# 3decomp/poissbox

Hardware: AMD Instinct MI355X
Metric: CG iter/s and DoF-updates/s at 512^3; achieved HBM GB/s vs peak (higher is better)
Workload: dtype f64

## Files before the change

poissbox_amd/csrc/pb_mg.cpp:

```cpp
#include <algorithm>
#include <cmath>

#include "pb_mg.hpp"

namespace pb {

int mg_plan_levels(const int64_t n[3], int nranks, int levels_req) {
  std::vector<int64_t> k0(nranks), nz(nranks);
  for (int r = 0; r < nranks; ++r) pb_slab_partition(n[2], nranks, r, &k0[r], &nz[r]);
  int64_t cur[3] = {n[0], n[1], n[2]};
  int L = 1;
  const int cap = levels_req > 0 ? levels_req : 64;
  while (L < cap) {
    bool ok = true;
    for (int d = 0; d < 3; ++d) ok = ok && cur[d] % 4 == 0;
    if (levels_req <= 0) ok = ok && std::min(cur[0], std::min(cur[1], cur[2])) > 4;
    for (int r = 0; r < nranks; ++r) ok = ok && k0[r] % 2 == 0 && nz[r] % 2 == 0;
    if (!ok) break;
    for (int d = 0; d < 3; ++d) cur[d] /= 2;
    for (int r = 0; r < nranks; ++r) {
      k0[r] /= 2;
      nz[r] /= 2;
    }
    ++L;
// ... 10 lines not shown
    if (L.own) pb_grid_destroy(L.g);
  if (mg->mem) (void)hipFree(mg->mem);
  if (mg->agg) (void)hipFree(mg->agg);
  if (mg->pmem) (void)hipFree(mg->pmem);
  if (mg->vmem) (void)hipFree(mg->vmem);
  delete mg;
}

static MgTune mg_tunings(const pb_ctx* ctx) {
  MgTune t;
  t.engine_min_plane = tune("mg_engine_min_plane", ctx->split ? 128 * 128 : 256 * 256);
  t.restrict_z_min_cols = tune("mg_restrict_z_min_cols", 4096);
  t.tail_max = tune("mg_tail_max", 8192);
  t.split_fused = tune("mg_split_fused", 1) != 0;
  t.poly_fused = tune("mg_poly_fused", 1) != 0;
  t.vc_pre_fused = tune("mg_varcoef_pre_fused", 1) != 0;
  t.vc_dinv_stored = tune("mg_varcoef_dinv_stored", 0) != 0;
  t.vc_kc = tune("mg_varcoef_kc", 0);
  return t;
}

static LevelPlan level_plan(const Mg* mg, int l, bool have_xs) {
  const MgTune& tn = mg->tn;
  const pb_grid* g = mg->lv[l].g;
  const bool split = mg->ctx->split;
  LevelPlan p;
  p.engine = g->plane >= tn.engine_min_plane;
  if (l + 1 >= (int)mg->lv.size()) return p;
  const pb_grid* c = mg->lv[l + 1].g;
  p.march = c->n[0] * c->n[1] >= tn.restrict_z_min_cols;
  if (mg->custom()) return p;
  const bool sweep2 = p.engine && sor_sweep2_supported(g);
  const bool u4 = sweep2 && (!split || (tn.split_fused && g->k0 % 2 == 0));
  if (u4 && g->nzl % 2 == 0 && (!split || g->nzl >= 3)) p.pre = LevelPlan::FusedRestrict;
  else if (sweep2) p.pre = LevelPlan::FusedResidual;
  if (u4 && have_xs && p.march && (!split || (g->nzl >= 2 && c->nzl >= 2)))
    p.post = LevelPlan::PostSweep;
  else if (sweep2 && p.march)
    p.post = LevelPlan::ProlongThenSweep2;
  return p;
}

static int tail_first(const Mg* mg) {
  const int L = (int)mg->lv.size();
  int Lt = L;
  for (int l = L - 1; l >= 1 && mg->lv[l].size() <= mg->tn.tail_max; --l) Lt = l;
  return L - Lt > kTailMax ? L : Lt;
}

static int mg_agglomerate_setup(Mg* mg) {
  pb_ctx* ctx = mg->ctx;
// ... 63 lines not shown
      lv.g = g;
      continue;
    }
    const int rc = grid_create_part(ctx, lv.n, g->L, g->k0 >> l, g->nzl >> l, &lv.g);
    if (rc != PB_OK) {
      mg_destroy(mg);
      return rc;
    }
    lv.own = true;
  }
  std::vector<double**> arrays;
  std::vector<int64_t> sizes;
  int64_t total = 0;
  for (int l = 0; l < L; ++l) {
    MgLevel& lv = mg->lv[l];
    const bool xs = level_plan(mg, l, true).post == LevelPlan::PostSweep;
    for (double** a : {l > 0 ? &lv.x : nullptr, l > 0 ? &lv.b : nullptr,
                       l < L - 1 ? &lv.res : nullptr, xs ? &lv.xs : nullptr}) {
      if (!a) continue;
      arrays.push_back(a);
      sizes.push_back(lv.g->nlocal);
      total += lv.g->nlocal;
    }
  }
  if (total > 0 && hipMalloc(&mg->mem, (size_t)total * sizeof(double)) != hipSuccess) {
    mg_destroy(mg);
    return set_error(PB_ERR_ALLOC, "multigrid levels: out of device memory");
  }
  double* p = mg->mem;
  for (size_t i = 0; i < arrays.size(); ++i) {
    *arrays[i] = p;
// ... 100 lines not shown
    PB_TRY(poly_step(mg, F, y, ypa, r, scale, omega, yo, ro));
    yp = y;
    y = yo;
    r = ro;
  }
  *ycur = const_cast<double*>(y);
  *rcur = const_cast<double*>(r);
  return PB_OK;
}

static int down_leg(Mg* mg, int l) {
  pb_ctx* ctx = mg->ctx;
  MgLevel& F = mg->lv[l];
  MgLevel& C = mg->lv[l + 1];
  const LevelPlan& p = F.plan;
  F.cur = p.post == LevelPlan::PostSweep ? F.xs : F.x;
  double* res = F.res;
  {
    ScopedTimer t1(ctx, l == 0 ? "mg_fine_smooth_first" : "mg_coarse_levels");
    if (p.pre == LevelPlan::FusedRestrict)
      return launch_presmooth_restrict(F.g, F.s, C.g, F.b, F.cur, C.b, mg->omega, mg->skip);
    if (p.pre == LevelPlan::FusedResidual) {
      PB_TRY(launch_presmooth_residual(F.g, F.s, F.b, F.cur, F.res, mg->omega, mg->skip));
    } else if (mg->poly()) {
      PB_TRY(poly_smooth(mg, F, true, &F.cur, &res));
    } else {
      PB_TRY(level_smooth(mg, F, 0, 1));
      for (int i = 1; i < mg->sm.nu; ++i) {
        PB_TRY(level_smooth(mg, F, 0, 0));
        PB_TRY(level_smooth(mg, F, 1, 0));
      }
// ... 85 lines not shown
```

poissbox_amd/csrc/pb_mg.hpp:

```cpp
#pragma once
#include <vector>

#include "pb_internal.hpp"

namespace pb {

struct MgGeo {
  int nx, ny, nzl;
  int64_t plane, nlocal, k0;
};

struct LevelPlan {
  enum Pre { FusedRestrict, FusedResidual, Sweeps };
  enum Post { PostSweep, ProlongThenSweep2, ProlongThenHalves };
  bool engine = false;
  Pre pre = Sweeps;
  Post post = ProlongThenHalves;
  bool march = false;
};

struct MgLevel {
  int64_t n[3];
  double h[3];
  Star s;
  pb_grid* g = nullptr;
  bool own = false;
  double* x = nullptr;
  double* b = nullptr;
  double* res = nullptr;
  double* xs = nullptr;
  double* t1 = nullptr;
  double* t2 = nullptr;
  double* r2 = nullptr;
// ... 3 lines not shown
  Star vs;
  LevelPlan plan;
  double* cur = nullptr;
  int64_t size() const { return n[0] * n[1] * n[2]; }
  MgGeo geo() const {
    return MgGeo{(int)g->n[0], (int)g->n[1], (int)g->nzl, g->plane, g->nlocal, g->k0};
  }
};

struct MgTune {
  int64_t engine_min_plane;
  int64_t restrict_z_min_cols;
  int64_t tail_max;
  bool split_fused;
  bool poly_fused;
  bool vc_pre_fused, vc_dinv_stored;
  int vc_kc;
};

struct MgSums {
  const CgState* st = nullptr;
  int* nparts = nullptr;
};

struct CoarsePlanes {
  const double *xc, *lo, *hi;
};

static constexpr int kTailMax = 12;

// ... 42 lines not shown
```

poissbox_amd/csrc/pb_mg_sweep.hip:

```cpp
#include <algorithm>
#include <type_traits>

#include "pb_device.hpp"

namespace pb {

#ifndef PB_SWEEP2_TY
#define PB_SWEEP2_TY 3
#endif
static constexpr int kTY2 = PB_SWEEP2_TY;
static constexpr int kRW = kTY2 + 4;
static constexpr int kSegOut = 112;
static constexpr int kSegLead = 4;

__device__ __forceinline__ double pick(bool e1, const double (&v)[2]) {
  const long long m = -(long long)e1;
  return __builtin_bit_cast(double, (__builtin_bit_cast(long long, v[1]) & m) |
                                        (__builtin_bit_cast(long long, v[0]) & ~m));
}

struct Sweep2Geo {
  int nx, ny, nzl;
  int64_t plane;
  int nseg, ntile, kc, nchunk;
// ... 362 lines not shown
      rq[0][r] = rq[1][r];
      rq[1][r] = rq[2][r];
      rq[2][r] = rn[r];
#pragma unroll
      for (int e = 0; e < 2; ++e) {
        s1[0][r][e] = s1[1][r][e];
        s1[1][r][e] = s1[2][r][e];
        bq[0][r][e] = bq[1][r][e];
        bq[1][r][e] = bq[2][r][e];
      }
    }
    keepb(nraw, bq[2]);
  }
}

template <int NW, int TY>
__device__ __forceinline__ void presmooth_restrict_u4_range(
    const Sweep2Geo& g, int ncx, int64_t cplane, double cx, double cy, double cz, double cc,
    double omega, const double* __restrict__ b, double* __restrict__ xout,
    double* __restrict__ bc, int seg, int tile, int kb, int ke, double (&xch)[2][8][NW][64]) {
  static_assert(TY % 2 == 0 && TY >= 2, "whole coarse rows per wave");
  constexpr int RB = NW * TY;
  constexpr int LO = 4;
  constexpr int SB = RB - 2 * LO;
  constexpr int NCR = TY / 2;
  const double icc = 1.0 / cc;
  const int lane = threadIdx.x & 63, wid = __builtin_amdgcn_readfirstlane(threadIdx.x >> 6);
  const int nx = g.nx, ny = g.ny, nz = g.nzl;
  if (kb >= nz) return;
  const int g0 = tile * SB - LO;
  const int br0 = wid * TY;
// ... 141 lines not shown
          a = a + cx * xl;
          a = a + cc * s1c[r][e];
          a = a + cx * xr;
          a = a + cy * yp;
          a = a + cz * s1p[r][e];
          rv[e] = bq0[r][e] - a;
        }
        const double rlo = dpp_from_lower(rv[1]);
        const double rhi = dpp_from_upper(rv[0]);
        double sx = w[0] * rlo;
        sx = sx + w[1] * rv[0];
        sx = sx + w[2] * rv[1];
        sx = sx + w[3] * rhi;
        sxc[r] = sx;
      }
      if (k >= kb && k < ke && out_ok) {
        const int64_t base = (int64_t)k * g.plane;
#pragma unroll
        for (int r = 0; r < TY; ++r)
          if (row_ok >> r & 1u) store_row<2>(xout, rix(base + ro[r]), s1c[r], g.nt);
      }
    } else {
#pragma unroll
      for (int r = 0; r < TY; ++r) sxc[r] = 0.0;
    }
    xch[KP][6][wid][lane] = sxc[0];
    xch[KP][7][wid][lane] = sxc[TY - 1];
    const int kr = k - 1;
    if (kr >= kb - 1) {
#pragma unroll
      for (int c = 0; c < NCR; ++c) {
        double sy = 0.0;
#pragma unroll
        for (int bb = 0; bb < 4; ++bb) {
          const int r = 2 * c - 1 + bb;
// ... 15 lines not shown
      }
    }
    redv(std::integral_constant<int, KP ^ 1>{}, raw, rn);
    xch[KP][0][wid][lane] = rn[0];
    xch[KP][1][wid][lane] = rn[TY - 1];
  };
#pragma unroll 1
  for (int k = kb - 3; k <= ke + 1; k += 4) {
    body(std::integral_constant<int, 0>{}, k);
    body(std::integral_constant<int, 1>{}, k + 1);
    body(std::integral_constant<int, 2>{}, k + 2);
    body(std::integral_constant<int, 3>{}, k + 3);
  }
}

template <class F>
__device__ __forceinline__ void split_ranges(const Sweep2Geo& g, int bid, F&& fn) {
  const int ncol = g.nseg * g.ntile, W = g.wsplit, T = g.nzl / W;
  if (bid < T * ncol) {
    const int kb = (bid / ncol) * W;
    fn(bid % ncol, kb, kb + W);
    return;
  }
  const int k0 = T * W, h = g.nzl - k0;
  if (h <= 0) return;
  const int64_t total = (int64_t)ncol * h;
  const int64_t e = min(total, (int64_t)(bid - T * ncol + 1) * W);
  for (int64_t s = (int64_t)(bid - T * ncol) * W; s < e;) {
    const int col = (int)(s / h);
    const int kb = (int)(s - (int64_t)col * h);
    const int ke = (int)min((int64_t)h, kb + (e - s));
    fn(col, k0 + kb, k0 + ke);
    s += ke - kb;
  }
}

template <int NW, int TY>
__global__ __launch_bounds__(64 * NW) void presmooth_restrict_u4_kernel(
    Sweep2Geo g, int ncx, int64_t cplane, double cx, double cy, double cz, double cc,
    double omega, const double* __restrict__ b, double* __restrict__ xout,
    double* __restrict__ bc, const int* skip) {
  __shared__ double xch[2][8][NW][64];
  if (skip && *skip) return;
  int bid = xcd_block(g.remap);
  if (g.wsplit > 0) {
    split_ranges(g, bid, [&](int col, int kb, int ke) {
      presmooth_restrict_u4_range<NW, TY>(g, ncx, cplane, cx, cy, cz, cc, omega, b, xout, bc,
                                          col % g.nseg, col / g.nseg, kb, ke, xch);
      __syncthreads();
    });
    return;
  }
  const int seg = bid % g.nseg;
  bid /= g.nseg;
  const int tile = bid % g.ntile;
  const int chunk = bid / g.ntile;
  const int kb = chunk * g.kc;
  presmooth_restrict_u4_range<NW, TY>(g, ncx, cplane, cx, cy, cz, cc, omega, b, xout, bc, seg,
                                      tile, kb, min(kb + g.kc, g.nzl), xch);
}

struct PostGeo {
  int ncx, ncy, ncz;
  int64_t cplane;
  int split;
  const double* cgh[4];
};

template <bool SUMS, int NW, int TY>
__device__ __forceinline__ void post_sweep_u4_range(
    const Sweep2Geo& g, const PostGeo& cgeo, double cx, double cy, double cz, double cc,
    double omega, const double* __restrict__ xs, const double* __restrict__ xc,
    const double* __restrict__ b, double* __restrict__ xout, double mu, int seg, int tile, int kb,
    int ke, double (&xch)[2][6][NW][64], double (&acc)[4]) {
  static_assert(TY % 2 == 0 && TY >= 2, "own rows start on an even fine row");
  constexpr int RB = NW * TY;
  constexpr int SB = RB - 4;
  constexpr int NC = TY / 2 + 2;
  const double icc = 1.0 / cc;
  const int lane = threadIdx.x & 63, wid = __builtin_amdgcn_readfirstlane(threadIdx.x >> 6);
  const int nx = g.nx, ny = g.ny, nz = g.nzl;
  if (kb < nz) {
    const int g0 = tile * SB - 2;
    const int br0 = wid * TY;
    const int j0 = g0 + br0;
    auto wrap = [](int v, int n) { v %= n; return v < 0 ? v + n : v; };
    int ip = seg * kSegOut + 2 * (lane - kSegLead);
    if (ip < 0) ip += nx;
    if (ip >= nx) ip -= nx;
    const int o = seg * kSegOut + 2 * (lane - kSegLead);
    const bool out_ok = lane >= kSegLead && lane < kSegLead + kSegOut / 2 && o < nx;
    int64_t ro[TY];
    unsigned row_ok = 0;
#pragma unroll
    for (int r = 0; r < TY; ++r) {
      ro[r] = (int64_t)wrap(j0 + r, ny) * nx;
      const int brow = br0 + r;
      if (brow >= 2 && brow < RB - 2 && g0 + brow < ny) row_ok |= 1u << r;
    }
    const unsigned boff = (unsigned)ip * 8u;
    auto rix = [&](int64_t row) { return RowIx{row, boff}; };
    auto wrapk = [&](int kk) { kk %= nz; return kk < 0 ? kk + nz : kk; };
    auto pl = [&](int kk) -> int64_t { return (int64_t)wrapk(kk) * g.plane; };
    int64_t crow[NC];
#pragma unroll
    for (int t = 0; t < NC; ++t) crow[t] = (int64_t)wrap((j0 >> 1) - 1 + t, cgeo.ncy) * cgeo.ncx;
    const unsigned cboff = (unsigned)(ip >> 1) * 8u;
    auto xsplane = [&](int kk) -> const double* {
      if (!g.split) return xs + pl(kk);
      if (kk >= 0 && kk < nz) return xs + (int64_t)kk * g.plane;
      const int gi = kk < 0 ? max(kk + 2, 0) : 2 + min(kk - nz, 1);
      return g.xg + (int64_t)gi * g.plane;
    };
    auto ldx = [&](double (&dst)[TY + 2][2], int kk) {
      const double* src = xsplane(kk);
#pragma unroll
      for (int r = 0; r < TY; ++r) load_row<2>(src, rix(ro[r]), dst[r + 1]);
    };
    auto ldc = [&](double (&cv)[NC], int K) {
      const double* cp;
      if (!cgeo.split) {
        K %= cgeo.ncz;
        if (K < 0) K += cgeo.ncz;
        cp = xc + (int64_t)K * cgeo.cplane;
      } else if (K >= 0 && K < cgeo.ncz) {
        cp = xc + (int64_t)K * cgeo.cplane;
      } else {
        const int gi = K < 0 ? max(K + 2, 0) : 2 + min(K - cgeo.ncz, 1);
        cp = cgeo.cgh[gi];
      }
#pragma unroll
      for (int t = 0; t < NC; ++t)
        cv[t] = *reinterpret_cast<const double*>(reinterpret_cast<const char*>(cp + crow[t]) + cboff);
    };
    auto yinterp = [&](const double (&cv)[NC], double (&Y)[TY][2]) {
      double xi[NC][2];
#pragma unroll
      for (int t = 0; t < NC; ++t) {
        const double c = cv[t];
        xi[t][0] = 0.75 * c + 0.25 * dpp_from_lower(c);
        xi[t][1] = 0.75 * c + 0.25 * dpp_from_upper(c);
      }
#pragma unroll
      for (int r = 0; r < TY; ++r) {
        const int tJ = 1 + (r >> 1);
        const int tf = (r & 1) ? tJ + 1 : tJ - 1;
#pragma unroll
        for (int e = 0; e < 2; ++e) Y[r][e] = 0.75 * xi[tJ][e] + 0.25 * xi[tf][e];
      }
    };
    auto prolong = [&](double (&v)[TY + 2][2], const double (&Yn)[TY][2],
                       const double (&Yf)[TY][2]) {
#pragma unroll
      for (int r = 0; r < TY; ++r)
#pragma unroll
        for (int e = 0; e < 2; ++e) v[r + 1][e] = v[r + 1][e] + (0.75 * Yn[r][e] + 0.25 * Yf[r][e]);
    };
    auto ldb = [&](double (&dst)[TY][2], int kk) {
      const double* src = !g.split ? b + pl(kk)
                          : (kk >= 0 && kk < nz ? b + (int64_t)kk * g.plane
                                                : (kk < 0 ? g.bg_lo : g.bg_hi));
#pragma unroll
      for (int r = 0; r < TY; ++r) load_row<2>(src, rix(ro[r]), dst[r]);
    };
    auto e1 = [](int r, int P) { return ((r + P) & 1) ^ 1; };
    auto half1 = [&](auto Pc, const double (&zmv)[TY], const double (&xcn)[TY + 2][2],
                     const double (&xp)[TY + 2][2], const double (&bb)[TY][2],
                     double (&out)[TY]) {
      constexpr int P = decltype(Pc)::value;
#pragma unroll
      for (int r = 0; r < TY; ++r) {
        const int e = e1(r, P);
        const double xl = e ? xcn[r + 1][0] : dpp_from_lower(xcn[r + 1][1]);
        const double xr = e ? dpp_from_upper(xcn[r + 1][0]) : xcn[r + 1][1];
        double nb = cz * zmv[r];
        nb = nb + cy * xcn[r][e];
        nb = nb + cx * xl;
        nb = nb + cx * xr;
        nb = nb + cy * xcn[r + 2][e];
        nb = nb + cz * xp[r + 1][e];
        const double t = (bb[r][e] - nb) * icc;
        out[r] = (1.0 - omega) * xcn[r + 1][e] + omega * t;
      }
    };
    auto half2 = [&](auto Pc, int kk, const double (&sm)[TY], const double (&sc)[TY],
                     const double (&sp)[TY], const double (&sh)[2], const double (&xo)[TY],
                     const double (&bo)[TY], const double (&bc1)[SUMS ? TY : 1]) {
      constexpr int P = decltype(Pc)::value;
      const int64_t base = pl(kk);
#pragma unroll
      for (int r = 0; r < TY; ++r) {
        const int e2 = e1(r, P) ^ 1;
        const double cself = sc[r];
        const double xl = e2 ? cself : dpp_from_lower(cself);
        const double xr = e2 ? dpp_from_upper(cself) : cself;
        double nb = cz * sm[r];
        nb = nb + cy * (r == 0 ? sh[0] : sc[r == 0 ? 0 : r - 1]);
        nb = nb + cx * xl;
        nb = nb + cx * xr;
        nb = nb + cy * (r == TY - 1 ? sh[1] : sc[r == TY - 1 ? r : r + 1]);
        nb = nb + cz * sp[r];
        const double t = (bo[r] - nb) * icc;
        const double v = (1.0 - omega) * xo[r] + omega * t;
        double ov[2];
        ov[e2] = v;
        ov[e2 ^ 1] = cself;
        if (out_ok && (row_ok >> r & 1u)) {
          store_row<2>(xout, rix(base + ro[r]), ov, g.nt);
          if constexpr (SUMS) {
            double rv2[2];
            rv2[e2] = bo[r];
            rv2[e2 ^ 1] = bc1[r];
#pragma unroll
            for (int e = 0; e < 2; ++e) {
              const double t2 = ov[e] - mu;
              acc[0] += t2;
              acc[1] += t2 * t2;
              acc[2] += t2 * rv2[e];
              acc[3] += rv2[e];
            }
          }
        }
      }
    };
    const int wm = wid > 0 ? wid - 1 : wid, wp = wid < NW - 1 ? wid + 1 : wid;
    auto put_x = [&](int par, const double (&v)[TY + 2][2]) {
      xch[par][0][wid][lane] = v[1][0];
      xch[par][1][wid][lane] = v[1][1];
      xch[par][2][wid][lane] = v[TY][0];
      xch[par][3][wid][lane] = v[TY][1];
    };
    double XQ[2][TY + 2][2];
    double XM[2][TY];
    double S1[4][TY];
    double SH[2][2];
    double BB[2][TY];
    double BB1[2][SUMS ? TY : 1];
    double YC[2][TY][2];
    const int K0 = kb >> 1;
    {
      double cv[NC];
      ldc(cv, K0 - 2);
      yinterp(cv, YC[0]);
      ldc(cv, K0 - 1);
      yinterp(cv, YC[1]);
      ldx(XQ[1], kb - 2);
      prolong(XQ[1], YC[1], YC[0]);
#pragma unroll
      for (int r = 0; r < TY; ++r) XM[1][r] = XQ[1][r + 1][e1(r, 0) ^ 1];
      ldc(cv, K0);
      yinterp(cv, YC[0]);
      ldx(XQ[0], kb - 1);
      prolong(XQ[0], YC[1], YC[0]);
      put_x(1, XQ[0]);
    }
#pragma unroll
    for (int r = 0; r < TY; ++r) {
      XM[0][r] = BB[0][r] = BB[1][r] = 0.0;
      S1[0][r] = S1[1][r] = S1[2][r] = 0.0;
      if constexpr (SUMS) BB1[0][r] = BB1[1][r] = 0.0;
    }
    SH[0][0] = SH[0][1] = 0.0;
    auto body = [&](auto Qc, int k) {
      constexpr int Q = decltype(Qc)::value;
      constexpr int KP = Q & 1;
      double (&xq1)[TY + 2][2] = XQ[Q & 1];
      double (&xq2)[TY + 2][2] = XQ[(Q + 1) & 1];
      double (&xm)[TY] = XM[Q & 1];
      double (&x0)[TY] = XM[(Q + 1) & 1];
      double (&bm)[TY] = BB[Q & 1];
      double (&bm1)[SUMS ? TY : 1] = BB1[Q & 1];
      double (&shp)[2] = SH[Q & 1];
      double (&shc)[2] = SH[(Q + 1) & 1];
      constexpr int KN = Q >> 1;
      double bq1[TY][2], cv[NC];
      ldx(xq2, k + 2);
      if constexpr (Q & 1) ldc(cv, ((k + 2) >> 1) + 1);
      ldb(bq1, k + 1);
      __syncthreads();
      {
        constexpr int rp = KP ^ 1;
        xq1[0][0] = xch[rp][2][wm][lane];
        xq1[0][1] = xch[rp][3][wm][lane];
        xq1[TY + 1][0] = xch[rp][0][wp][lane];
        xq1[TY + 1][1] = xch[rp][1][wp][lane];
        shc[0] = xch[rp][5][wm][lane];
        shc[1] = xch[rp][4][wp][lane];
      }
      if (k > kb && k <= ke)
        half2(std::integral_constant<int, KP ^ 1>{}, k - 1, S1[Q], S1[(Q + 1) & 3],
              S1[(Q + 2) & 3], shp, xm, bm, bm1);
      if constexpr (Q & 1) yinterp(cv, YC[KN ^ 1]);
      prolong(xq2, YC[KN], YC[KN ^ 1]);
      put_x(KP, xq2);
      double (&s1n)[TY] = S1[(Q + 3) & 3];
      half1(std::integral_constant<int, KP ^ 1>{}, x0, xq1, xq2, bq1, s1n);
      xch[KP][4][wid][lane] = s1n[0];
      xch[KP][5][wid][lane] = s1n[TY - 1];
#pragma unroll
      for (int r = 0; r < TY; ++r) {
        const int e = e1(r, KP ^ 1);
        xm[r] = xq1[r + 1][e ^ 1];
        bm[r] = bq1[r][e ^ 1];
        if constexpr (SUMS) bm1[r] = bq1[r][e];
      }
    };
#pragma unroll 1
    for (int k = kb - 2; k <= ke; k += 4) {
      body(std::integral_constant<int, 0>{}, k);
      body(std::integral_constant<int, 1>{}, k + 1);
      body(std::integral_constant<int, 2>{}, k + 2);
      body(std::integral_constant<int, 3>{}, k + 3);
    }
  }
}

template <bool SUMS, int NW, int TY>
__global__ __launch_bounds__(64 * NW) void post_sweep_u4_kernel(
    Sweep2Geo g, PostGeo cgeo, double cx, double cy, double cz, double cc, double omega,
    const double* __restrict__ xs, const double* __restrict__ xc, const double* __restrict__ b,
    double* __restrict__ xout, const CgState* st, double* parts, const int* skip) {
  __shared__ double xch[2][6][NW][64];
  if (skip && *skip) return;
  double acc[4] = {0.0, 0.0, 0.0, 0.0};
  const double mu = SUMS ? st->mu : 0.0;
  int bid = xcd_block(g.remap);
  if (g.wsplit > 0) {
    split_ranges(g, bid, [&](int col, int kb, int ke) {
      post_sweep_u4_range<SUMS, NW, TY>(g, cgeo, cx, cy, cz, cc, omega, xs, xc, b, xout, mu,
                                        col % g.nseg, col / g.nseg, kb, ke, xch, acc);
      __syncthreads();
    });
  } else {
    const int seg = bid % g.nseg;
    bid /= g.nseg;
    const int tile = bid % g.ntile;
    const int chunk = bid / g.ntile;
    const int kb = chunk * g.kc;
    post_sweep_u4_range<SUMS, NW, TY>(g, cgeo, cx, cy, cz, cc, omega, xs, xc, b, xout, mu, seg,
                                      tile, kb, min(kb + g.kc, g.nzl), xch, acc);
  }
  if constexpr (SUMS) block_partials<4>(acc, parts);
}

bool sor_sweep2_supported(const pb_grid* g) {
  return g->n[0] >= 128 && g->n[0] % 2 == 0 && g->n[1] % 2 == 0 && g->n[1] >= 8 &&
         g->nzl >= 4 && tune("mg_sweep2", 1) != 0;
}

static int ensure_ghost2(pb_grid* g) {
  if (!g->ghost2 && hipMalloc(&g->ghost2, 6 * (size_t)g->plane * sizeof(double)) != hipSuccess)
    return set_error(PB_ERR_ALLOC, "deep ghost planes: out of device memory");
  return PB_OK;
}

// ... 91 lines not shown
  if (g->k0 % 2 != 0) return set_error(PB_ERR_UNSUPPORTED, "%s: odd slab origin", what);
  sweep2_geo(g, geo);
  geo.split = 0;
  geo.xg = geo.bg_lo = geo.bg_hi = nullptr;
  geo.ntile = (geo.ny + rows - 1) / rows;
  return PB_OK;
}

int launch_post_sweep(pb_grid* g, const Star& s, const pb_grid* cg, const double* xs,
                      const double* xc, const double* b, double* xout, double omega,
                      const int* skip, const CgState* sums_st, int* nparts,
                      const double* xc_full) {
  ScopedTimer tm(g->ctx, "mg_post_sweep");
  const bool split = g->ctx->split;
  if (xs == xout) return set_error(PB_ERR_ARG, "fused post-smoothing must run out of place");
  constexpr int nw = 8, ty = 4;
  Sweep2Geo geo;
  PB_TRY(u4_setup("fused post-smoothing", g, cg, 2, "fused post-smoothing: slabs of < 2 planes",
                  nw * ty - 4, geo));
  PostGeo cgeo{(int)cg->n[0], (int)cg->n[1], (int)cg->nzl, cg->plane, 0,
                {nullptr, nullptr, nullptr, nullptr}};
  if (split) {
    pb_grid* gc = const_cast<pb_grid*>(cg);
    PB_TRY(ensure_ghost2(g));
    PB_TRY(ensure_ghost2(gc));
    PB_TRY(halo_exchange_n(g, xs, xs + (g->nzl - 2) * g->plane, 2, g->ghost2,
                           g->ghost2 + 2 * g->plane));
    PB_TRY(halo_exchange(g, b, b + (g->nzl - 1) * g->plane));
    geo.split = 1;
    geo.xg = g->ghost2;
// ... 9 lines not shown
    } else {
      PB_TRY(halo_exchange_n(gc, xc, xc + (gc->nzl - 2) * gc->plane, 2, gc->ghost2,
                             gc->ghost2 + 2 * gc->plane));
      for (int i = 0; i < 4; ++i) cgeo.cgh[i] = gc->ghost2 + (int64_t)i * gc->plane;
    }
  }
  const int columns = geo.nseg * geo.ntile;
  const int target = 8 * g->ctx->num_cus;
  int nchunk = std::max(1, (target + columns - 1) / columns);
  const int minz = std::min(64, std::max(16, geo.nzl / 8));
  nchunk = std::min(nchunk, std::max(1, geo.nzl / minz));
  int64_t nblocks = set_chunks(geo, nchunk, 4);
  nblocks = balanced_split(g, geo, std::max(0, tune("mg_u4_split", 0)), 4, nblocks);
  double* parts;
  PB_TRY(sums_parts(g, sums_st, nblocks, nparts, &parts));
  auto kern = sums_st ? post_sweep_u4_kernel<true, nw, ty> : post_sweep_u4_kernel<false, nw, ty>;
  hipLaunchKernelGGL(kern, dim3((unsigned)nblocks), dim3(64 * nw), 0, g->ctx->stream, geo, cgeo,
                     s.cx, s.cy, s.cz, s.cc, omega, xs, xc, b, xout, sums_st, parts, skip);
  PB_HIP(hipGetLastError());
  return PB_OK;
}

int launch_presmooth_restrict(pb_grid* g, const Star& s, const pb_grid* cg, const double* b,
                              double* xout, double* bc, double omega, const int* skip) {
  ScopedTimer tm(g->ctx, "mg_presmooth_restrict");
  const bool split = g->ctx->split;
  if (b == xout) return set_error(PB_ERR_ARG, "fused pre-smoothing must run out of place");
  if (!sor_sweep2_supported(g) || g->nzl % 2)
    return set_error(PB_ERR_UNSUPPORTED, "fused restriction: grid not supported");
  constexpr int nw = 8, ty = 4;
  Sweep2Geo geo;
// ... 2 lines not shown
  if (split) {
    PB_TRY(ensure_ghost2(g));
    PB_TRY(halo_exchange_n(g, b, b + (g->nzl - 3) * g->plane, 3, g->ghost2,
                           g->ghost2 + 3 * g->plane));
    geo.split = 1;
    geo.xg = g->ghost2;
  }
  const int columns = geo.nseg * geo.ntile;
  int nchunk = std::max(1, g->ctx->num_cus / columns);
  if (geo.nzl / nchunk < 128) nchunk = std::max(1, (4 * g->ctx->num_cus + columns - 1) / columns);
  nchunk = std::min(nchunk, std::max(1, geo.nzl / 16));
  int64_t nblocks = set_chunks(geo, nchunk, 2);
  const int ps = tune("mg_u4_split", -1);
  nblocks = balanced_split(g, geo, ps >= 0 ? ps : (nblocks > g->ctx->num_cus ? 1 : 0), 2,
                           nblocks);
  hipLaunchKernelGGL((presmooth_restrict_u4_kernel<nw, ty>), dim3((unsigned)nblocks),
                     dim3(64 * nw), 0, g->ctx->stream, geo, (int)cg->n[0], cg->plane, s.cx, s.cy,
                     s.cz, s.cc, omega, b, xout, bc, skip);
  PB_HIP(hipGetLastError());
  return PB_OK;
}

int launch_presmooth_residual(pb_grid* g, const Star& s, const double* b, double* x, double* res,
                              double omega, const int* skip) {
  ScopedTimer tm(g->ctx, "mg_presmooth_residual");
  if (b == x || b == res || x == res)
    return set_error(PB_ERR_ARG, "fused pre-smoothing + residual must run out of place");
  Sweep2Geo geo;
  const int64_t nblocks = sweep2_geo(g, geo);
  PB_TRY(sweep2_ghosts(g, b, b, geo));
  auto kern = geo.split ? presmooth_resid_kernel<true> : presmooth_resid_kernel<false>;
  hipLaunchKernelGGL(kern, dim3((unsigned)nblocks), dim3(kThreads), 0, g->ctx->stream, geo,
                     s.cx, s.cy, s.cz, s.cc, omega, b, x, res, skip);
// ... 6 lines not shown
```

poissbox_amd/csrc/pb_runtime.cpp:

```cpp
#include <time.h>

#include <algorithm>
#include <atomic>
#include <chrono>
#include <cstdarg>
#include <cstdlib>
#include <cstring>
#include <condition_variable>
#include <memory>
#include <mutex>
#include <string>
#include <thread>
#include <unordered_map>

#include "pb_internal.hpp"

namespace pb {

hipError_t field_alloc(void** p, size_t bytes) { return hipMalloc(p, bytes); }

void field_free(void* p) {
  if (p) (void)hipFree(p);
}

namespace {
const char* const kTuneNames[] = {
    "a2a_copy_self", "cg_defer_x", "engine_kc_skew", "cg_fold", "cg_fuse", "cg_sr_fused", "cheb_fused", "comm_mark_every",
    "comm_stall_test_ms", "compact_lines", "fft_rupd", "fgmres_fused", "pipecg_fused", "fft_zpad", "fft_zpad_min_plane",
    "force_comm", "ksp_lazy0", "mg_agglomerate", "mg_engine_min_plane", "mg_poly_fused", "mg_restrict_z_min_cols",
    "mg_split_fused", "mg_sweep2", "mg_tail_max", "mg_u4_split", "mg_varcoef_dinv_stored", "mg_varcoef_kc",
    "mg_varcoef_pre_fused", "pcr_lines", "rich_fused", "sor_omega_any", "sr_ddiff",
    "stencil_kc", "stencil_kc_skew", "stencil_nt", "stencil_tall", "stencil_wgcu", "varcoef_dot_fused", "varcoef_wgcu", "x_dot_cu"};
constexpr int kNumTune = (int)(sizeof(kTuneNames) / sizeof(kTuneNames[0]));
std::atomic<int> g_tune_val[kNumTune];
std::atomic<int> g_tune_set[kNumTune];
std::atomic<int> g_tune_nset{0};
int tune_index(const char* name) {
  for (int i = 0; i < kNumTune; ++i)
    if (strcmp(kTuneNames[i], name) == 0) return i;
  return -1;
}
}

int tune(const char* name, int dflt) {
// ... 1019 lines not shown
```

Before: 102.4 billion.

## Recompute pre-smoothed iterate in post-sweep instead of storing it

On single-rank levels using the fused presmooth+restrict path, the pre-smoothed iterate x_s is no longer written to memory. The post-sweep kernel instead rebuilds it from b, since x starts at zero and one red-black sweep pass can be re-derived locally. This removes one full-grid store and one full-grid load per level per V-cycle and also frees the x_s buffer. In exchange the post-sweep does more arithmetic, more LDS exchange and an extra staging buffer, with scalar-load tricks to limit register pressure.

```diff
diff --git a/poissbox_amd/csrc/pb_mg.cpp b/poissbox_amd/csrc/pb_mg.cpp
--- a/poissbox_amd/csrc/pb_mg.cpp
+++ b/poissbox_amd/csrc/pb_mg.cpp
@@ -48,6 +48,7 @@
   t.tail_max = tune("mg_tail_max", 8192);
   t.split_fused = tune("mg_split_fused", 1) != 0;
   t.poly_fused = tune("mg_poly_fused", 1) != 0;
+  t.recompute_xs = tune("mg_recompute_xs", 1) != 0;
   t.vc_pre_fused = tune("mg_varcoef_pre_fused", 1) != 0;
   t.vc_dinv_stored = tune("mg_varcoef_dinv_stored", 0) != 0;
   t.vc_kc = tune("mg_varcoef_kc", 0);
@@ -68,7 +69,8 @@
   const bool u4 = sweep2 && (!split || (tn.split_fused && g->k0 % 2 == 0));
   if (u4 && g->nzl % 2 == 0 && (!split || g->nzl >= 3)) p.pre = LevelPlan::FusedRestrict;
   else if (sweep2) p.pre = LevelPlan::FusedResidual;
-  if (u4 && have_xs && p.march && (!split || (g->nzl >= 2 && c->nzl >= 2)))
+  p.recompute_xs = tn.recompute_xs && u4 && !split && p.pre == LevelPlan::FusedRestrict && p.march;
+  if (u4 && (have_xs || p.recompute_xs) && p.march && (!split || (g->nzl >= 2 && c->nzl >= 2)))
     p.post = LevelPlan::PostSweep;
   else if (sweep2 && p.march)
     p.post = LevelPlan::ProlongThenSweep2;
@@ -162,7 +164,8 @@
   int64_t total = 0;
   for (int l = 0; l < L; ++l) {
     MgLevel& lv = mg->lv[l];
-    const bool xs = level_plan(mg, l, true).post == LevelPlan::PostSweep;
+    const LevelPlan lp = level_plan(mg, l, true);
+    const bool xs = lp.post == LevelPlan::PostSweep && !lp.recompute_xs;
     for (double** a : {l > 0 ? &lv.x : nullptr, l > 0 ? &lv.b : nullptr,
                        l < L - 1 ? &lv.res : nullptr, xs ? &lv.xs : nullptr}) {
       if (!a) continue;
@@ -293,7 +296,7 @@
   MgLevel& F = mg->lv[l];
   MgLevel& C = mg->lv[l + 1];
   const LevelPlan& p = F.plan;
-  F.cur = p.post == LevelPlan::PostSweep ? F.xs : F.x;
+  F.cur = p.post == LevelPlan::PostSweep ? (p.recompute_xs ? nullptr : F.xs) : F.x;
   double* res = F.res;
   {
     ScopedTimer t1(ctx, l == 0 ? "mg_fine_smooth_first" : "mg_coarse_levels");
diff --git a/poissbox_amd/csrc/pb_mg.hpp b/poissbox_amd/csrc/pb_mg.hpp
--- a/poissbox_amd/csrc/pb_mg.hpp
+++ b/poissbox_amd/csrc/pb_mg.hpp
@@ -17,6 +17,7 @@
   Pre pre = Sweeps;
   Post post = ProlongThenHalves;
   bool march = false;
+  bool recompute_xs = false;
 };
 
 struct MgLevel {
@@ -50,6 +51,7 @@
   int64_t tail_max;
   bool split_fused;
   bool poly_fused;
+  bool recompute_xs;
   bool vc_pre_fused, vc_dinv_stored;
   int vc_kc;
 };
diff --git a/poissbox_amd/csrc/pb_mg_sweep.hip b/poissbox_amd/csrc/pb_mg_sweep.hip
--- a/poissbox_amd/csrc/pb_mg_sweep.hip
+++ b/poissbox_amd/csrc/pb_mg_sweep.hip
@@ -400,7 +400,7 @@
   }
 }
 
-template <int NW, int TY>
+template <bool STORE, int NW, int TY>
 __device__ __forceinline__ void presmooth_restrict_u4_range(
     const Sweep2Geo& g, int ncx, int64_t cplane, double cx, double cy, double cz, double cc,
     double omega, const double* __restrict__ b, double* __restrict__ xout,
@@ -572,11 +572,13 @@
         sx = sx + w[3] * rhi;
         sxc[r] = sx;
       }
-      if (k >= kb && k < ke && out_ok) {
-        const int64_t base = (int64_t)k * g.plane;
-#pragma unroll
-        for (int r = 0; r < TY; ++r)
-          if (row_ok >> r & 1u) store_row<2>(xout, rix(base + ro[r]), s1c[r], g.nt);
+      if constexpr (STORE) {
+        if (k >= kb && k < ke && out_ok) {
+          const int64_t base = (int64_t)k * g.plane;
+#pragma unroll
+          for (int r = 0; r < TY; ++r)
+            if (row_ok >> r & 1u) store_row<2>(xout, rix(base + ro[r]), s1c[r], g.nt);
+        }
       }
     } else {
 #pragma unroll
@@ -622,7 +624,7 @@
   }
 }
 
-template <class F>
+template <bool PER_RANGE = false, class F>
 __device__ __forceinline__ void split_ranges(const Sweep2Geo& g, int bid, F&& fn) {
   const int ncol = g.nseg * g.ntile, W = g.wsplit, T = g.nzl / W;
   if (bid < T * ncol) {
@@ -630,11 +632,13 @@
     fn(bid % ncol, kb, kb + W);
     return;
   }
-  const int k0 = T * W, h = g.nzl - k0;
+  const int k0 = T * W;
+  int h = g.nzl - k0;
   if (h <= 0) return;
   const int64_t total = (int64_t)ncol * h;
   const int64_t e = min(total, (int64_t)(bid - T * ncol + 1) * W);
   for (int64_t s = (int64_t)(bid - T * ncol) * W; s < e;) {
+    if constexpr (PER_RANGE) asm volatile("" : "+s"(h));
     const int col = (int)(s / h);
     const int kb = (int)(s - (int64_t)col * h);
     const int ke = (int)min((int64_t)h, kb + (e - s));
@@ -643,7 +647,7 @@
   }
 }
 
-template <int NW, int TY>
+template <bool STORE, int NW, int TY>
 __global__ __launch_bounds__(64 * NW) void presmooth_restrict_u4_kernel(
     Sweep2Geo g, int ncx, int64_t cplane, double cx, double cy, double cz, double cc,
     double omega, const double* __restrict__ b, double* __restrict__ xout,
@@ -653,7 +657,7 @@
   int bid = xcd_block(g.remap);
   if (g.wsplit > 0) {
     split_ranges(g, bid, [&](int col, int kb, int ke) {
-      presmooth_restrict_u4_range<NW, TY>(g, ncx, cplane, cx, cy, cz, cc, omega, b, xout, bc,
+      presmooth_restrict_u4_range<STORE, NW, TY>(g, ncx, cplane, cx, cy, cz, cc, omega, b, xout, bc,
                                           col % g.nseg, col / g.nseg, kb, ke, xch);
       __syncthreads();
     });
@@ -664,7 +668,7 @@
   const int tile = bid % g.ntile;
   const int chunk = bid / g.ntile;
   const int kb = chunk * g.kc;
-  presmooth_restrict_u4_range<NW, TY>(g, ncx, cplane, cx, cy, cz, cc, omega, b, xout, bc, seg,
+  presmooth_restrict_u4_range<STORE, NW, TY>(g, ncx, cplane, cx, cy, cz, cc, omega, b, xout, bc, seg,
                                       tile, kb, min(kb + g.kc, g.nzl), xch);
 }
 
@@ -675,17 +679,30 @@
   const double* cgh[4];
 };
 
-template <bool SUMS, int NW, int TY>
+static constexpr int post_xch_slots(bool rx) { return rx ? 8 : 6; }
+static constexpr int post_park_len(bool rx, int nw, int ty) { return rx ? 2 * ty * 2 * nw * 64 : 1; }
+
+template <bool SUMS, bool RX, int NW, int TY>
 __device__ __forceinline__ void post_sweep_u4_range(
     const Sweep2Geo& g, const PostGeo& cgeo, double cx, double cy, double cz, double cc,
     double omega, const double* __restrict__ xs, const double* __restrict__ xc,
     const double* __restrict__ b, double* __restrict__ xout, double mu, int seg, int tile, int kb,
-    int ke, double (&xch)[2][6][NW][64], double (&acc)[4]) {
+    int ke, double (&xch)[2][post_xch_slots(RX)][NW][64],
+    double (&park)[post_park_len(RX, NW, TY)], double (&acc)[4]) {
   static_assert(TY % 2 == 0 && TY >= 2, "own rows start on an even fine row");
+  static_assert(!RX || (NW >= 2 && kSegLead >= 3), "recomputed x_s: two end waves, three halo pairs");
   constexpr int RB = NW * TY;
   constexpr int SB = RB - 4;
   constexpr int NC = TY / 2 + 2;
   const double icc = 1.0 / cc;
+  auto sdouble = [](double v) {
+    if constexpr (!RX) return v;
+    const unsigned long long u = __builtin_bit_cast(unsigned long long, v);
+    const unsigned lo = __builtin_amdgcn_readfirstlane((unsigned)u);
+    const unsigned hi = __builtin_amdgcn_readfirstlane((unsigned)(u >> 32));
+    return __builtin_bit_cast(double, ((unsigned long long)hi << 32) | lo);
+  };
+  const double om1 = sdouble(1.0 - omega), om1z = sdouble((1.0 - omega) * 0.0);
   const int lane = threadIdx.x & 63, wid = __builtin_amdgcn_readfirstlane(threadIdx.x >> 6);
   const int nx = g.nx, ny = g.ny, nz = g.nzl;
   if (kb < nz) {
@@ -708,7 +725,38 @@
     }
     const unsigned boff = (unsigned)ip * 8u;
     auto rix = [&](int64_t row) { return RowIx{row, boff}; };
-    auto wrapk = [&](int kk) { kk %= nz; return kk < 0 ? kk + nz : kk; };
+    auto srow = [](const double* p) {
+      const unsigned long long a = reinterpret_cast<unsigned long long>(p);
+      const unsigned lo = __builtin_amdgcn_readfirstlane((unsigned)a);
+      const unsigned hi = __builtin_amdgcn_readfirstlane((unsigned)(a >> 32));
+      return ((unsigned long long)hi << 32) | lo;
+    };
+    auto ld1_s = [](unsigned long long row, unsigned off) {
+      return *(const __attribute__((address_space(1))) double*)(row + off);
+    };
+    auto ld2_s = [](unsigned long long row, unsigned off, double (&v)[2]) {
+      const dv2 t = *(const __attribute__((address_space(1))) dv2*)(row + off);
+      v[0] = t.x;
+      v[1] = t.y;
+    };
+    auto st2_s = [](unsigned long long row, unsigned off, const double (&v)[2], int nt) {
+      dv2 t;
+      t.x = v[0];
+      t.y = v[1];
+      auto* q = (__attribute__((address_space(1))) dv2*)(row + off);
+      if (nt) __builtin_nontemporal_store(t, q);
+      else *q = t;
+    };
+    auto wrap3 = [](int v, int n) {
+      v = v < 0 ? v + n : v;
+      v = v >= n ? v - n : v;
+      return v >= n ? v - n : v;
+    };
+    auto wrapk = [&](int kk) {
+      if constexpr (RX) return wrap3(kk, nz);
+      kk %= nz;
+      return kk < 0 ? kk + nz : kk;
+    };
     auto pl = [&](int kk) -> int64_t { return (int64_t)wrapk(kk) * g.plane; };
     int64_t crow[NC];
 #pragma unroll
@@ -727,7 +775,9 @@
     };
     auto ldc = [&](double (&cv)[NC], int K) {
       const double* cp;
-      if (!cgeo.split) {
+      if (RX) {
+        cp = xc + (int64_t)wrap3(K, cgeo.ncz) * cgeo.cplane;
+      } else if (!cgeo.split) {
         K %= cgeo.ncz;
         if (K < 0) K += cgeo.ncz;
         cp = xc + (int64_t)K * cgeo.cplane;
@@ -738,8 +788,11 @@
         cp = cgeo.cgh[gi];
       }
 #pragma unroll
-      for (int t = 0; t < NC; ++t)
-        cv[t] = *reinterpret_cast<const double*>(reinterpret_cast<const char*>(cp + crow[t]) + cboff);
+      for (int t = 0; t < NC; ++t) {
+        const double* rowp = cp + crow[t];
+        if constexpr (RX) cv[t] = ld1_s(srow(rowp), cboff);
+        else cv[t] = *reinterpret_cast<const double*>(reinterpret_cast<const char*>(rowp) + cboff);
+      }
     };
     auto yinterp = [&](const double (&cv)[NC], double (&Y)[TY][2]) {
       double xi[NC][2];
@@ -769,10 +822,54 @@
                           : (kk >= 0 && kk < nz ? b + (int64_t)kk * g.plane
                                                 : (kk < 0 ? g.bg_lo : g.bg_hi));
 #pragma unroll
-      for (int r = 0; r < TY; ++r) load_row<2>(src, rix(ro[r]), dst[r]);
+      for (int r = 0; r < TY; ++r) {
+        if constexpr (RX) ld2_s(srow(src + ro[r]), boff, dst[r]);
+        else load_row<2>(src, rix(ro[r]), dst[r]);
+      }
     };
     auto e1 = [](int r, int P) { return ((r + P) & 1) ^ 1; };
-    auto half1 = [&](auto Pc, const double (&zmv)[TY], const double (&xcn)[TY + 2][2],
+    auto redval = [&](double bv) {
+      const double t = (bv - 0.0) * icc;
+      return om1z + omega * t;
+    };
+    auto redv = [&](auto Pc, const double (&v)[TY][2], double (&red)[TY]) {
+      constexpr int P = decltype(Pc)::value;
+#pragma unroll
+      for (int r = 0; r < TY; ++r) red[r] = redval(v[r][e1(r, P) ^ 1]);
+    };
+    auto xs_form = [&](auto Pc, auto Red, const double (&rm)[TY], const double (&rc)[TY],
+                       const double (&rp)[TY], const double (&rh)[2], const double (&bb)[TY][2],
+                       double (&out)[TY + 2][2]) {
+      constexpr int P = decltype(Pc)::value;
+#pragma unroll
+      for (int r = 0; r < TY; ++r) {
+        const int be = e1(r, P);
+        const double xl = be ? rc[r] : dpp_from_lower(rc[r]);
+        const double xr = be ? dpp_from_upper(rc[r]) : rc[r];
+        double nb = cz * rm[r];
+        nb = nb + cy * (r == 0 ? rh[0] : rc[r == 0 ? 0 : r - 1]);
+        nb = nb + cx * xl;
+        nb = nb + cx * xr;
+        nb = nb + cy * (r == TY - 1 ? rh[1] : rc[r == TY - 1 ? r : r + 1]);
+        nb = nb + cz * rp[r];
+        const double t = (bb[r][be] - nb) * icc;
+        const double v = om1z + omega * t;
+        if constexpr (decltype(Red)::value) out[r + 1][1 - be] = rc[r];
+        out[r + 1][be] = v;
+      }
+    };
+    const int64_t exrow =
+        (int64_t)wrap(wid == 0 ? j0 - 1 : (wid == NW - 1 ? j0 + TY : j0), ny) * nx;
+    auto ldex = [&](auto Pc, int kk) {
+      constexpr int P = decltype(Pc)::value;
+      const int e = P ? (wid == NW - 1 ? 1 : 0) : (wid == 0 ? 1 : 0);
+      return ld1_s(srow(b + pl(kk) + exrow + e), boff);
+    };
+    auto red_halo = [&](double (&rh)[2], double lo, double hi, double ex) {
+      rh[0] = wid == 0 ? redval(ex) : lo;
+      rh[1] = wid == NW - 1 ? redval(ex) : hi;
+    };
+    auto half1 =[&](auto Pc, const double (&zmv)[TY], const double (&xcn)[TY + 2][2],
                      const double (&xp)[TY + 2][2], const double (&bb)[TY][2],
                      double (&out)[TY]) {
       constexpr int P = decltype(Pc)::value;
@@ -788,7 +885,7 @@
         nb = nb + cy * xcn[r + 2][e];
         nb = nb + cz * xp[r + 1][e];
         const double t = (bb[r][e] - nb) * icc;
-        out[r] = (1.0 - omega) * xcn[r + 1][e] + omega * t;
+        out[r] = om1 * xcn[r + 1][e] + omega * t;
       }
     };
     auto half2 = [&](auto Pc, int kk, const double (&sm)[TY], const double (&sc)[TY],
@@ -809,12 +906,13 @@
         nb = nb + cy * (r == TY - 1 ? sh[1] : sc[r == TY - 1 ? r : r + 1]);
         nb = nb + cz * sp[r];
         const double t = (bo[r] - nb) * icc;
-        const double v = (1.0 - omega) * xo[r] + omega * t;
+        const double v = om1 * xo[r] + omega * t;
         double ov[2];
         ov[e2] = v;
         ov[e2 ^ 1] = cself;
         if (out_ok && (row_ok >> r & 1u)) {
-          store_row<2>(xout, rix(base + ro[r]), ov, g.nt);
+          if constexpr (RX) st2_s(srow(xout + base + ro[r]), boff, ov, g.nt);
+          else store_row<2>(xout, rix(base + ro[r]), ov, g.nt);
           if constexpr (SUMS) {
             double rv2[2];
             rv2[e2] = bo[r];
@@ -845,6 +943,7 @@
     double BB[2][TY];
     double BB1[2][SUMS ? TY : 1];
     double YC[2][TY][2];
+    double BQ[RX ? 4 : 1][TY][2];
     const int K0 = kb >> 1;
     {
       double cv[NC];
@@ -852,13 +951,39 @@
       yinterp(cv, YC[0]);
       ldc(cv, K0 - 1);
       yinterp(cv, YC[1]);
-      ldx(XQ[1], kb - 2);
+      if constexpr (RX) {
+        std::integral_constant<int, 0> ev;
+        std::integral_constant<int, 1> od;
+        double r3[TY], r2[TY], r1[TY], r0[TY], rh2[2], rh1[2];
+        ldb(BQ[2], kb - 3);
+        ldb(BQ[3], kb - 2);
+        ldb(BQ[0], kb - 1);
+        ldb(BQ[1], kb);
+        const double ex2 = ldex(ev, kb - 2), ex1 = ldex(od, kb - 1);
+        redv(od, BQ[2], r3);
+        redv(ev, BQ[3], r2);
+        redv(od, BQ[0], r1);
+        redv(ev, BQ[1], r0);
+        xch[0][6][wid][lane] = r2[0];
+        xch[0][7][wid][lane] = r2[TY - 1];
+        xch[0][4][wid][lane] = r1[0];
+        xch[0][5][wid][lane] = r1[TY - 1];
+        xch[1][6][wid][lane] = r0[0];
+        xch[1][7][wid][lane] = r0[TY - 1];
+        __syncthreads();
+        red_halo(rh2, xch[0][7][wm][lane], xch[0][6][wp][lane], ex2);
+        red_halo(rh1, xch[0][5][wm][lane], xch[0][4][wp][lane], ex1);
+        xs_form(ev, std::true_type{}, r3, r2, r1, rh2, BQ[3], XQ[1]);
+        xs_form(od, std::true_type{}, r2, r1, r0, rh1, BQ[0], XQ[0]);
+      } else {
+        ldx(XQ[1], kb - 2);
+      }
       prolong(XQ[1], YC[1], YC[0]);
 #pragma unroll
       for (int r = 0; r < TY; ++r) XM[1][r] = XQ[1][r + 1][e1(r, 0) ^ 1];
       ldc(cv, K0);
       yinterp(cv, YC[0]);
-      ldx(XQ[0], kb - 1);
+      if constexpr (!RX) ldx(XQ[0], kb - 1);
       prolong(XQ[0], YC[1], YC[0]);
       put_x(1, XQ[0]);
     }
@@ -881,12 +1006,21 @@
       double (&shp)[2] = SH[Q & 1];
       double (&shc)[2] = SH[(Q + 1) & 1];
       constexpr int KN = Q >> 1;
-      double bq1[TY][2], cv[NC];
-      ldx(xq2, k + 2);
+      double bql[RX ? 1 : TY][2], cv[NC];
+      double (&bq1)[TY][2] = *[&]() {
+        if constexpr (RX) return &BQ[Q];
+        else return &bql;
+      }();
+      double ex = 0.0, rh[2] = {0.0, 0.0};
+      if constexpr (RX) {
+        ldb(BQ[(Q + 2) & 3], k + 3);
+      } else {
+        ldx(xq2, k + 2);
+      }
       if constexpr (Q & 1) ldc(cv, ((k + 2) >> 1) + 1);
-      ldb(bq1, k + 1);
+      if constexpr (!RX) ldb(bq1, k + 1);
       __syncthreads();
-      {
+      auto get_halos = [&]() {
         constexpr int rp = KP ^ 1;
         xq1[0][0] = xch[rp][2][wm][lane];
         xq1[0][1] = xch[rp][3][wm][lane];
@@ -894,23 +1028,76 @@
         xq1[TY + 1][1] = xch[rp][1][wp][lane];
         shc[0] = xch[rp][5][wm][lane];
         shc[1] = xch[rp][4][wp][lane];
-      }
-      if (k > kb && k <= ke)
+      };
+      if constexpr (!RX) get_halos();
+      if constexpr (RX) {
+        if (k > kb && k <= ke) {
+          double pb2[TY], pb1[SUMS ? TY : 1];
+#pragma unroll
+          for (int r = 0; r < TY; ++r) {
+            pb2[r] = park[(((Q & 1) * TY + r) * 2 + 0) * (NW * 64) + threadIdx.x];
+            if constexpr (SUMS) pb1[r] = park[(((Q & 1) * TY + r) * 2 + 1) * (NW * 64) + threadIdx.x];
+          }
+          half2(std::integral_constant<int, KP ^ 1>{}, k - 1, S1[Q], S1[(Q + 1) & 3],
+                S1[(Q + 2) & 3], shp, xm, pb2, pb1);
+        }
+      } else if (k > kb && k <= ke) {
         half2(std::integral_constant<int, KP ^ 1>{}, k - 1, S1[Q], S1[(Q + 1) & 3],
               S1[(Q + 2) & 3], shp, xm, bm, bm1);
-      if constexpr (Q & 1) yinterp(cv, YC[KN ^ 1]);
-      prolong(xq2, YC[KN], YC[KN ^ 1]);
-      put_x(KP, xq2);
+      }
       double (&s1n)[TY] = S1[(Q + 3) & 3];
-      half1(std::integral_constant<int, KP ^ 1>{}, x0, xq1, xq2, bq1, s1n);
-      xch[KP][4][wid][lane] = s1n[0];
-      xch[KP][5][wid][lane] = s1n[TY - 1];
-#pragma unroll
-      for (int r = 0; r < TY; ++r) {
-        const int e = e1(r, KP ^ 1);
-        xm[r] = xq1[r + 1][e ^ 1];
-        bm[r] = bq1[r][e ^ 1];
-        if constexpr (SUMS) bm1[r] = bq1[r][e];
+      if constexpr (RX) {
+        __builtin_amdgcn_sched_barrier(0);
+        if constexpr (Q & 1) yinterp(cv, YC[KN ^ 1]);
+        const double (&Yn)[TY][2] = YC[KN];
+        const double (&Yf)[TY][2] = YC[KN ^ 1];
+        double rm[TY], rc[TY], rn[TY];
+        redv(std::integral_constant<int, KP>{}, BQ[(Q + 1) & 3], rc);
+#pragma unroll
+        for (int r = 0; r < TY; ++r) {
+          const int re = e1(r, KP) ^ 1;
+          xq2[r + 1][re] = rc[r] + (0.75 * Yn[r][re] + 0.25 * Yf[r][re]);
+        }
+        get_halos();
+        ex = ldex(std::integral_constant<int, KP>{}, k + 2);
+        half1(std::integral_constant<int, KP ^ 1>{}, x0, xq1, xq2, bq1, s1n);
+        xch[KP][4][wid][lane] = s1n[0];
+        xch[KP][5][wid][lane] = s1n[TY - 1];
+        redv(std::integral_constant<int, KP ^ 1>{}, bq1, rm);
+#pragma unroll
+        for (int r = 0; r < TY; ++r) {
+          const int e = e1(r, KP ^ 1);
+          xm[r] = xq1[r + 1][e ^ 1];
+          park[(((Q & 1) * TY + r) * 2 + 0) * (NW * 64) + threadIdx.x] = bq1[r][e ^ 1];
+          if constexpr (SUMS) park[(((Q & 1) * TY + r) * 2 + 1) * (NW * 64) + threadIdx.x] = bq1[r][e];
+        }
+        __builtin_amdgcn_sched_barrier(0);
+        red_halo(rh, xch[KP ^ 1][7][wm][lane], xch[KP ^ 1][6][wp][lane], ex);
+        redv(std::integral_constant<int, KP ^ 1>{}, BQ[(Q + 2) & 3], rn);
+        xch[KP][6][wid][lane] = rn[0];
+        xch[KP][7][wid][lane] = rn[TY - 1];
+        xs_form(std::integral_constant<int, KP>{}, std::false_type{}, rm, rc, rn, rh,
+                BQ[(Q + 1) & 3], xq2);
+#pragma unroll
+        for (int r = 0; r < TY; ++r) {
+          const int be = e1(r, KP);
+          xq2[r + 1][be] = xq2[r + 1][be] + (0.75 * Yn[r][be] + 0.25 * Yf[r][be]);
+        }
+        put_x(KP, xq2);
+      } else {
+        if constexpr (Q & 1) yinterp(cv, YC[KN ^ 1]);
+        prolong(xq2, YC[KN], YC[KN ^ 1]);
+        put_x(KP, xq2);
+        half1(std::integral_constant<int, KP ^ 1>{}, x0, xq1, xq2, bq1, s1n);
+        xch[KP][4][wid][lane] = s1n[0];
+        xch[KP][5][wid][lane] = s1n[TY - 1];
+#pragma unroll
+        for (int r = 0; r < TY; ++r) {
+          const int e = e1(r, KP ^ 1);
+          xm[r] = xq1[r + 1][e ^ 1];
+          bm[r] = bq1[r][e ^ 1];
+          if constexpr (SUMS) bm1[r] = bq1[r][e];
+        }
       }
     };
 #pragma unroll 1
@@ -923,20 +1110,23 @@
   }
 }
 
-template <bool SUMS, int NW, int TY>
+template <bool SUMS, bool RX, int NW, int TY>
 __global__ __launch_bounds__(64 * NW) void post_sweep_u4_kernel(
     Sweep2Geo g, PostGeo cgeo, double cx, double cy, double cz, double cc, double omega,
     const double* __restrict__ xs, const double* __restrict__ xc, const double* __restrict__ b,
     double* __restrict__ xout, const CgState* st, double* parts, const int* skip) {
-  __shared__ double xch[2][6][NW][64];
+  __shared__ double xch[2][post_xch_slots(RX)][NW][64];
+  __shared__ double park[post_park_len(RX, NW, TY)];
   if (skip && *skip) return;
   double acc[4] = {0.0, 0.0, 0.0, 0.0};
   const double mu = SUMS ? st->mu : 0.0;
   int bid = xcd_block(g.remap);
   if (g.wsplit > 0) {
-    split_ranges(g, bid, [&](int col, int kb, int ke) {
-      post_sweep_u4_range<SUMS, NW, TY>(g, cgeo, cx, cy, cz, cc, omega, xs, xc, b, xout, mu,
-                                        col % g.nseg, col / g.nseg, kb, ke, xch, acc);
+    split_ranges<RX>(g, bid, [&](int col, int kb, int ke) {
+      int nseg = g.nseg;
+      if constexpr (RX) asm volatile("" : "+s"(nseg));
+      post_sweep_u4_range<SUMS, RX, NW, TY>(g, cgeo, cx, cy, cz, cc, omega, xs, xc, b, xout, mu,
+                                            col % nseg, col / nseg, kb, ke, xch, park, acc);
       __syncthreads();
     });
   } else {
@@ -945,8 +1135,8 @@
     const int tile = bid % g.ntile;
     const int chunk = bid / g.ntile;
     const int kb = chunk * g.kc;
-    post_sweep_u4_range<SUMS, NW, TY>(g, cgeo, cx, cy, cz, cc, omega, xs, xc, b, xout, mu, seg,
-                                      tile, kb, min(kb + g.kc, g.nzl), xch, acc);
+    post_sweep_u4_range<SUMS, RX, NW, TY>(g, cgeo, cx, cy, cz, cc, omega, xs, xc, b, xout, mu, seg,
+                                      tile, kb, min(kb + g.kc, g.nzl), xch, park, acc);
   }
   if constexpr (SUMS) block_partials<4>(acc, parts);
 }
@@ -1068,6 +1258,8 @@
   ScopedTimer tm(g->ctx, "mg_post_sweep");
   const bool split = g->ctx->split;
   if (xs == xout) return set_error(PB_ERR_ARG, "fused post-smoothing must run out of place");
+  if (!xs && split)
+    return set_error(PB_ERR_UNSUPPORTED, "fused post-smoothing without x_s: one rank only");
   constexpr int nw = 8, ty = 4;
   Sweep2Geo geo;
   PB_TRY(u4_setup("fused post-smoothing", g, cg, 2, "fused post-smoothing: slabs of < 2 planes",
@@ -1107,7 +1299,10 @@
   nblocks = balanced_split(g, geo, std::max(0, tune("mg_u4_split", 0)), 4, nblocks);
   double* parts;
   PB_TRY(sums_parts(g, sums_st, nblocks, nparts, &parts));
-  auto kern = sums_st ? post_sweep_u4_kernel<true, nw, ty> : post_sweep_u4_kernel<false, nw, ty>;
+  auto kern = xs ? (sums_st ? post_sweep_u4_kernel<true, false, nw, ty>
+                            : post_sweep_u4_kernel<false, false, nw, ty>)
+                 : (sums_st ? post_sweep_u4_kernel<true, true, nw, ty>
+                            : post_sweep_u4_kernel<false, true, nw, ty>);
   hipLaunchKernelGGL(kern, dim3((unsigned)nblocks), dim3(64 * nw), 0, g->ctx->stream, geo, cgeo,
                      s.cx, s.cy, s.cz, s.cc, omega, xs, xc, b, xout, sums_st, parts, skip);
   PB_HIP(hipGetLastError());
@@ -1140,9 +1335,10 @@
   const int ps = tune("mg_u4_split", -1);
   nblocks = balanced_split(g, geo, ps >= 0 ? ps : (nblocks > g->ctx->num_cus ? 1 : 0), 2,
                            nblocks);
-  hipLaunchKernelGGL((presmooth_restrict_u4_kernel<nw, ty>), dim3((unsigned)nblocks),
-                     dim3(64 * nw), 0, g->ctx->stream, geo, (int)cg->n[0], cg->plane, s.cx, s.cy,
-                     s.cz, s.cc, omega, b, xout, bc, skip);
+  auto kern = xout ? presmooth_restrict_u4_kernel<true, nw, ty>
+                   : presmooth_restrict_u4_kernel<false, nw, ty>;
+  hipLaunchKernelGGL(kern, dim3((unsigned)nblocks), dim3(64 * nw), 0, g->ctx->stream, geo,
+                     (int)cg->n[0], cg->plane, s.cx, s.cy, s.cz, s.cc, omega, b, xout, bc, skip);
   PB_HIP(hipGetLastError());
   return PB_OK;
 }
diff --git a/poissbox_amd/csrc/pb_runtime.cpp b/poissbox_amd/csrc/pb_runtime.cpp
--- a/poissbox_amd/csrc/pb_runtime.cpp
+++ b/poissbox_amd/csrc/pb_runtime.cpp
@@ -27,7 +27,7 @@
 const char* const kTuneNames[] = {
     "a2a_copy_self", "cg_defer_x", "engine_kc_skew", "cg_fold", "cg_fuse", "cg_sr_fused", "cheb_fused", "comm_mark_every",
     "comm_stall_test_ms", "compact_lines", "fft_rupd", "fgmres_fused", "pipecg_fused", "fft_zpad", "fft_zpad_min_plane",
-    "force_comm", "ksp_lazy0", "mg_agglomerate", "mg_engine_min_plane", "mg_poly_fused", "mg_restrict_z_min_cols",
+    "force_comm", "ksp_lazy0", "mg_agglomerate", "mg_engine_min_plane", "mg_poly_fused", "mg_recompute_xs", "mg_restrict_z_min_cols",
     "mg_split_fused", "mg_sweep2", "mg_tail_max", "mg_u4_split", "mg_varcoef_dinv_stored", "mg_varcoef_kc",
     "mg_varcoef_pre_fused", "pcr_lines", "rich_fused", "sor_omega_any", "sr_ddiff",
     "stencil_kc", "stencil_kc_skew", "stencil_nt", "stencil_tall", "stencil_wgcu", "varcoef_dot_fused", "varcoef_wgcu", "x_dot_cu"};
```

Result: slower. 101.1 billion (-1.3%).
